# phylo42/RAPPAS

Measured on AMD Instinct MI355X. Metric: reads placed/sec (whole node), 150 bp DNA vs 10^7-kmer DB, higher is better.
Workload: dtype f32; 1 GPU; C2: DNA k=10, 999 branches, phylo-kmer DB of 786432 keys / 9995042 entries (seed 42), replicated per GPU; 10000000 x 150 symbol reads per GPU per step (uniform, seed 1+rank), keep_at_most=7; reads_per_gpu=10000000

## Files before the change

### rappas_amd/csrc/rk_engine.hip

```cpp
#include "rk_kernels.hip"
#include "rk_internal.h"
#include "rk_pack_host.h"
#include "rk_translate_host.h"
#include "rk_plan.h"
#include "rk_geometry.h"

#include <cmath>
#include <cstdarg>
#include <cstdio>
#include <cstdlib>
#include <algorithm>
#include <array>
#include <chrono>
#include <condition_variable>
#include <cstring>
#include <cerrno>
#include <cstddef>
#include <deque>
#include <functional>
#include <map>
#include <set>
#include <memory>
#include <atomic>
#include <mutex>
// ... 785 lines not shown
    }
    CL_TRY(hipDeviceSynchronize());
#undef CL_TRY
    db->compact_nib = src->compact_nib;
    finish_db(db, meta, src->info.table_mode, src->indexed, src->view.mono != 0, src->info.n_keys, src->info.n_entries, src->info.table_slots,
              src->view.hash_mask, table_bytes, blob_bytes, src->info.max_row_len);
    db->lanes_per_read = src->lanes_per_read;
    *out = db;
    return RK_OK;
    RK_GUARD_END("rk_db_clone")
}

extern "C" int rk_db_get_info(const rk_db *db, rk_db_info *info) {
    if (!db || !info) return fail(RK_ERR_INVALID, "rk_db_get_info: null argument");
    *info = db->info;
    return RK_OK;
}

extern "C" void *rk_host_alloc(uint64_t bytes) {
    void *p = nullptr;
    hipError_t e = hipHostMalloc(&p, bytes ? bytes : 1, hipHostMallocDefault);
    if (e != hipSuccess) {
        (void)fail(e == hipErrorOutOfMemory ? RK_ERR_NOMEM : RK_ERR_HIP, "rk_host_alloc(%llu) failed: %s", (unsigned long long)bytes, hipGetErrorString(e));
        return nullptr;
    }
    return p;
}

extern "C" void rk_host_free(void *p) {
    if (p) (void)hipHostFree(p);
}

extern "C" uint32_t rk_packed_words(const rk_db *db, uint32_t max_len) {
    if (!db) return 0;
    uint64_t bits = (uint64_t)max_len * db->info.bits_per_symbol;
    uint32_t w = (uint32_t)((bits + 31) / 32);
    return w ? w : 1;
}

extern "C" int rk_set_lanes_per_read(rk_db *db, uint32_t lanes) {
    if (!db) return fail(RK_ERR_INVALID, "rk_set_lanes_per_read: null db");
    if (lanes != 0 && lanes != 8 && lanes != 16 && lanes != 32 && lanes != 64)
        return fail(RK_ERR_INVALID, "rk_set_lanes_per_read: lanes must be 0 (auto), 8, 16, 32 or 64");
    if (lanes != 0 && db->indexed)
        return fail(RK_ERR_UNSUPPORTED, "rk_set_lanes_per_read: this database uses the large-tree image (n_branches > %u, long rows): always the workgroup-per-read kernel", RK_WG_MIN_BRANCHES);
    db->lanes_per_read = lanes;
    return RK_OK;
}

static int geometry_error(rk_geom::Status st, const rk_db *db, uint32_t keep_at_most = 0, size_t lds_per_read = 0) {
    switch (st) {
    case rk_geom::GEOM_OK: return RK_OK;
    case rk_geom::KEEP_NEEDS_LANES: return fail(RK_ERR_INVALID, "keep_at_most=%u needs lanes_per_read >= %u", keep_at_most, keep_at_most);
    case rk_geom::READ_EXCEEDS_LDS: return fail(RK_ERR_UNSUPPORTED, "n_branches=%u needs %zu B of LDS per read, more than one CU has (%zu B)", db->info.n_branches, lds_per_read, db->lds_per_cu);
    case rk_geom::NO_WG_WINDOW: return fail(RK_ERR_UNSUPPORTED, "n_branches=%u: no score-vector window fits one CU's LDS (%zu B)", db->info.n_branches, db->lds_per_cu);
    case rk_geom::WINDOWED_NO_FIT: return fail(RK_ERR_UNSUPPORTED, "internal: windowed geometry does not fit the LDS");
    default: return fail(RK_ERR_INVALID, "internal: ambiguity kernel launched without a score-vector geometry");
    }
}
static int db_geometry(const rk_db *db, uint32_t keep_at_most, Geometry &g) {
    const rk_geom::Status st = rk_geom::choose_geometry(db->info.n_branches, db->info.bits_per_symbol, db->lds_per_cu, db->lanes_per_read, keep_at_most, geom_knobs(), g);
    return geometry_error(st, db, keep_at_most, st == rk_geom::READ_EXCEEDS_LDS ? g.lds_per_wave : 0);
}
static int db_wg_geometry(const rk_db *db, WgGeometry &g, uint32_t keep_at_most = 16) {
    return geometry_error(rk_geom::choose_wg_geometry(db->info.n_branches, db->lds_per_cu, keep_at_most, geom_knobs(), g), db);
}

static bool use_pipelined16(const rk_db *db, const Geometry &g, const PlaceArgs &args) {
    static const bool off = rk_knob("RK_NO_PIPE") != nullptr;
    return !off && g.G == 16 && db->info.table_mode != RK_TABLE_HASH && db->info.rows_bytes < ROWS_FIT32_LIMIT && args.words_per_read <= 16;
}

template <int G, int BITS, int TM, bool WIDE>
static int launch_variant(const rk_db *db, const Geometry &g, const PlaceArgs &args, hipStream_t stream) {
    constexpr int PU = rk_geom::probe_unroll(G, BITS);
    constexpr int U = G == 64 ? RK_RING64 : RK_RING;
    auto kern = place_packed_kernel<G, BITS, TM, WIDE, U, PU>;
    decltype(kern) clade_kern = nullptr;
    PlaceArgs la = args;
    bool whole_simds = false;
    if constexpr (G == 16 && !WIDE && TM != TM_HASH) {
        if (use_pipelined16(db, g, args)) {
            whole_simds = TM == TM_COMPACT;
            auto k16 = place_packed16_kernel<BITS, TM, U, PU>;
            auto k24 = place_packed16_kernel<BITS, TM, U, PU, TM == TM_COMPACT>;
            if constexpr (BITS == 5) {
                if (!args.lens && args.fixed_len >= db->info.k && args.fixed_len - db->info.k + 1 <= 96u) {
                    k16 = place_packed16_kernel<BITS, TM, U, 6>;
                    k24 = place_packed16_kernel<BITS, TM, U, 6, TM == TM_COMPACT>;
                }
            }
            kern = k16;
            if (TM == TM_COMPACT && db->d_dense_rows) {
                kern = k24;
                la.db.compact = (const uint4 *)db->d_dense_table;
                la.db.rows = (const unsigned char *)db->d_dense_rows;
                la.db.rows_bytes = db->dense_rows_bytes;
                if (args.perm) {
                    clade_kern = k16;
                    la.only_if = 3u;
                }
            }
        }
    }
    const Grid grid{64, g.lds_per_wave, g.waves_per_cu, (args.n_reads + g.NG - 1) / g.NG, whole_simds};
    if (int rc = launch_grid(db->cu_count, kern, grid, stream, la)) return rc;
    if (!clade_kern) return RK_OK;
    PlaceArgs ca = args;
    ca.only_if = 4u;
    return launch_grid(db->cu_count, clade_kern, grid, stream, ca);
}

template <int G, int BITS>
static int launch_t(const rk_db *db, const Geometry &g, const PlaceArgs &a, hipStream_t s) {
    const bool wide = db->info.rows_bytes >= ROWS_FIT32_LIMIT;
    switch (db->info.table_mode) {
    case RK_TABLE_DIRECT: return wide ? launch_variant<G, BITS, TM_COMPACT, true>(db, g, a, s) : launch_variant<G, BITS, TM_COMPACT, false>(db, g, a, s);
    case RK_TABLE_DIRECT8: return wide ? launch_variant<G, BITS, TM_DIRECT8, true>(db, g, a, s) : launch_variant<G, BITS, TM_DIRECT8, false>(db, g, a, s);
    default: return wide ? launch_variant<G, BITS, TM_HASH, true>(db, g, a, s) : launch_variant<G, BITS, TM_HASH, false>(db, g, a, s);
    }
}
static bool use_windowed(const rk_db *db, uint32_t keep_at_most, uint32_t words_per_read) {
    static const bool off = rk_knob("RK_NO_WINDOW") != nullptr;
    const uint64_t max_symbols = (uint64_t)words_per_read * 32 / db->info.bits_per_symbol;
    const bool fits = words_per_read <= 16 || max_symbols * 9 <= db->info.n_branches || db->info.n_branches > 16000;
    return !off && db->windowed && db->lanes_per_read == 0 && keep_at_most <= 16 && fits;
}

static void *launch_scratch(const rk_db *db, hipStream_t s, size_t bytes) {
    std::lock_guard<std::mutex> lock(db->scratch_mu);
    rk_db::LaunchScratch *b = nullptr;
    for (auto &x : db->scratch)
        if (x.s == s) { b = &x; break; }
    if (!b) {
        if (db->scratch.size() >= 16) {
            auto lru = std::min_element(db->scratch.begin(), db->scratch.end(), [](const rk_db::LaunchScratch &x, const rk_db::LaunchScratch &y) { return x.used < y.used; });
            hipStreamCaptureStatus cs = hipStreamCaptureStatusNone;
            if (hipStreamIsCapturing(s, &cs) != hipSuccess || cs != hipStreamCaptureStatusNone || hipDeviceSynchronize() != hipSuccess) {
                (void)hipGetLastError();
                return nullptr;
            }
            if (lru->p) (void)hipFree(lru->p);
            db->scratch.erase(lru);
        }
        db->scratch.push_back({s, nullptr, 0, 0});
        b = &db->scratch.back();
    }
    b->used = ++db->scratch_clock;
    if (b->cap < bytes) {
        hipStreamCaptureStatus cs = hipStreamCaptureStatusNone;
        if (hipStreamIsCapturing(s, &cs) != hipSuccess || cs != hipStreamCaptureStatusNone) {
            (void)hipGetLastError();
            return nullptr;
        }
        if (b->p) {
            if (hipStreamSynchronize(s) != hipSuccess) { (void)hipGetLastError(); return nullptr; }
            (void)hipFree(b->p);
            b->p = nullptr;
            b->cap = 0;
        }
        const size_t want = ((bytes + bytes / 4) + ((size_t)1 << 20) - 1) & ~(((size_t)1 << 20) - 1);
        if (hipMalloc(&b->p, want) != hipSuccess || !b->p) {
            (void)hipGetLastError();
            b->p = nullptr;
            return nullptr;
        }
        b->cap = want;
    }
    return b->p;
}

struct TileOrder {
// ... 661 lines not shown
```

### rappas_amd/csrc/rk_geometry.h

```cpp
#pragma once
#include <cstddef>
#include <cstdint>
#include <initializer_list>
#include "rk_plan.h"

#ifndef RK_WG_MIN_BRANCHES
#define RK_WG_MIN_BRANCHES 8192u
#endif
#ifndef RK_WG_MIN_MEAN_ROW
#define RK_WG_MIN_MEAN_ROW 320.0
#endif
#ifndef RK_WG_ALWAYS_BRANCHES
#define RK_WG_ALWAYS_BRANCHES 65535u
#endif
#ifndef RK_WINDOW_MIN_BRANCHES
#define RK_WINDOW_MIN_BRANCHES 1276u
#endif
#ifndef RK_RING
#define RK_RING 8
#endif
#ifndef RK_RING64
#define RK_RING64 8
#endif

namespace rk_geom {

enum Status { GEOM_OK = 0, KEEP_NEEDS_LANES, READ_EXCEEDS_LDS, NO_WG_WINDOW, WINDOWED_NO_FIT, NO_SCORE_VECTOR };
struct Knobs {
    uint32_t list_cap = 0, waves_per_cu = 0;
    int wg_passes = 1;
    uint32_t hash_waves = ~0u;
    bool window_always = false, wstream_always = false;
};
constexpr uint32_t ROW_ENTRIES = 16;

static inline uint64_t resident_per_cu(uint64_t by_lds, uint64_t by_query, size_t lds) {
    uint64_t out = by_lds < by_query ? by_lds : by_query;
    if (lds) {
        const uint64_t by_granule = (160ull * 1024) / ((lds + 511) & ~(size_t)511);
        if (by_granule >= 1 && by_granule < out) out = by_granule;
    }
    return out;
}
static inline uint64_t grid_blocks(int cu_count, uint64_t per_cu, uint64_t work) { return (uint64_t)cu_count * per_cu > work ? work : (uint64_t)cu_count * per_cu; }

struct Geometry { uint32_t G, NG, s_stride, list_cap, pu; size_t lds_per_wave; uint32_t waves_per_cu; };
static constexpr uint32_t probe_unroll(uint32_t G, uint32_t bits) { return G <= 16 ? (bits == 5 && G == 16 ? 7 : 9) : (G == 32 ? 5 : 3); }
static inline Status choose_geometry(uint32_t nb, uint32_t bits, size_t lds_per_cu, uint32_t lanes_per_read, uint32_t keep_at_most, const Knobs &kn, Geometry &g) {
    const uint32_t s_stride = (nb + 4) & ~3u;
    const size_t target = lds_per_cu / 8;
    const size_t fixed = (size_t)s_stride * 4;
    auto bytes_for = [&](uint32_t G, uint32_t cap) { return (size_t)(64 / G) * (fixed + (size_t)cap * 8); };
    uint32_t G = lanes_per_read;
    if (G == 0) {
        G = 64;
        if (keep_at_most <= 16 && bytes_for(16, 16 + 3 * RK_RING + 40) <= lds_per_cu / 6) G = 16;
        else if (keep_at_most <= 32 && bytes_for(32, 32 + 3 * RK_RING + 40) <= lds_per_cu / 4) G = 32;
    }
    if (G < keep_at_most) return KEEP_NEEDS_LANES;
    const uint32_t NG = 64 / G, pu = probe_unroll(G, bits);
    const uint32_t min_cap = G + 3 * (G == 64 ? RK_RING64 : RK_RING) + 40;
    size_t per_group_target = target / NG;
    uint32_t cap = min_cap;
    if (per_group_target > fixed + (size_t)min_cap * 8) {
        size_t c = (per_group_target - fixed) / 8;
        cap = (uint32_t)(c > 256 ? 256 : c);
        if (cap < min_cap) cap = min_cap;
    }
    if (kn.list_cap >= min_cap && kn.list_cap <= 4096) cap = kn.list_cap;
    cap &= ~1u;
    g.G = G; g.NG = NG; g.s_stride = s_stride; g.list_cap = cap; g.pu = pu;
    g.lds_per_wave = bytes_for(G, cap);
    if (g.lds_per_wave > lds_per_cu) return READ_EXCEEDS_LDS;
    uint32_t w = (uint32_t)(lds_per_cu / g.lds_per_wave);
    g.waves_per_cu = w > 32 ? 32 : w;
    if (kn.waves_per_cu >= 1 && kn.waves_per_cu < g.waves_per_cu) g.waves_per_cu = kn.waves_per_cu;
    return GEOM_OK;
}

constexpr uint32_t RK_MAX_WINDOWS = 64;
static inline unsigned char winspec_byte(uint32_t first, uint32_t last) {
    const uint32_t span = last - first;
    return (unsigned char)(first | ((span < 3u ? span : 3u) << 6));
}
constexpr uint64_t RK_WINDOW_MAX_BLOB = 1ull << 31;
static inline bool windows_pay(uint32_t nb, uint64_t blob_units, uint64_t space, const Knobs &kn) {
    if (kn.window_always) return true;
    return 5 * blob_units <= 11 * space || nb > RK_WG_MIN_BRANCHES;
}
struct WindowPlan {
    uint32_t W = 0, n_win = 0, s_stride = 0, main_cap = 0, work_cap = 0;
    bool stream = false;
    double units_per_code = 0.0;
};
#ifndef RK_WSTREAM_MIN_BRANCHES
#define RK_WSTREAM_MIN_BRANCHES 4500u
#endif
static inline bool wstream_tree(uint32_t nb, uint32_t bits, double units_per_code, double units_per_row, const Knobs &kn) {
    if (kn.wstream_always) return true;
    if (150.0 * units_per_code > RK_WSTREAM_MAX_UNITS) return false;
    if (units_per_row > 2.5) return false;
    return bits == 5 || nb > RK_WSTREAM_MIN_BRANCHES;
}
static inline bool window_plan(uint32_t nb, uint32_t bits, double units_per_code, double units_per_row, const Knobs &kn, WindowPlan &wp) {
    if (nb <= RK_WINDOW_MIN_BRANCHES || nb > RK_WG_ALWAYS_BRANCHES) return false;
    wp.stream = wstream_tree(nb, bits, units_per_code, units_per_row, kn);
    wp.units_per_code = units_per_code;
    uint32_t n_win = wp.stream ? (nb + 511) / 512 : (nb + 895) / 896;
    if (n_win > RK_MAX_WINDOWS) n_win = RK_MAX_WINDOWS;
    wp.n_win = n_win;
    wp.W = ((nb + n_win - 1) / n_win + 3) & ~3u;
    wp.s_stride = wp.W + 4;
    const uint32_t per_group_words = 160 * 1024 / 8 / 4 / 4;
    const uint32_t avail = per_group_words - wp.s_stride;
    uint32_t work = avail > 256 + 88 ? avail - 256 : 88;
    if (work > 200) work = 200;
    wp.work_cap = work & ~1u;
    wp.main_cap = (avail - wp.work_cap) & ~1u;
    if (wp.main_cap > 640) wp.main_cap = 640;
    return wp.main_cap >= 160;
}
struct ImageKind { bool indexed, windowable; };
static inline ImageKind image_kind(uint32_t nb, uint32_t bits, bool direct, uint64_t space, uint64_t slot_units, uint32_t max_len, double mean_len, const Knobs &kn) {
    WindowPlan wp;
    const bool dense64_ahead = nb > RK_WG_MIN_BRANCHES && ((nb <= 9900u && mean_len >= 200.0 && mean_len < 1200.0) || (nb <= 13300u && mean_len >= 250.0 && mean_len < 750.0));
    const bool windowable = (!dense64_ahead || kn.window_always) && window_plan(nb, bits, space ? (double)slot_units / (double)space : 0.0, mean_len / ROW_ENTRIES + 0.5, kn, wp) && direct &&
                            (max_len + ROW_ENTRIES - 1) / ROW_ENTRIES <= 255 && slot_units * 128 < RK_WINDOW_MAX_BLOB && windows_pay(nb, slot_units, space, kn);
    const bool long_rows = mean_len >= RK_WG_MIN_MEAN_ROW;
    const bool indexed = nb > RK_WG_MIN_BRANCHES && ((long_rows && !dense64_ahead) || (!windowable && !dense64_ahead && nb > 16000u));
    return {indexed, windowable && !indexed};
}
struct WaveGeometry {
    uint32_t s_stride = 0, main_cap = 0, work_cap = 0, list_cap = 0, waves_cu = 0;
    size_t lds_wave = 0;
    bool wide = false;
};
static inline size_t lds_of_four_reads(uint32_t s_stride, uint32_t main_cap, uint32_t work_cap) { return (size_t)4 * (s_stride + main_cap + work_cap) * 4; }
static inline Status waves_that_fit(size_t lds_per_cu, uint32_t max_waves, WaveGeometry &o) {
    o.lds_wave = lds_of_four_reads(o.s_stride, o.main_cap, o.work_cap);
    o.waves_cu = (uint32_t)(lds_per_cu / o.lds_wave);
    if (o.waves_cu < 1) return WINDOWED_NO_FIT;
    if (o.waves_cu > max_waves) o.waves_cu = max_waves;
    return GEOM_OK;
}

static inline Status windowed_geometry(const WindowPlan &plan, uint32_t keep_at_most, uint32_t words_per_read, size_t lds_per_cu, WaveGeometry &o) {
    const uint32_t work_min = keep_at_most > 8 ? 96u : 88u;
    o.work_cap = plan.work_cap < work_min || words_per_read > 10 ? work_min : plan.work_cap;
    o.main_cap = plan.main_cap + plan.work_cap - o.work_cap;
    o.s_stride = plan.s_stride; o.list_cap = o.work_cap / 2;
    return waves_that_fit(lds_per_cu, 8u, o);
}

static inline bool sorted_wide(const WindowPlan &wp) { return wp.W > 512; }
static inline Status sorted_geometry(const WindowPlan &wp, size_t lds_per_cu, WaveGeometry &o) {
    const uint32_t work_min = 96u;
    const uint32_t ring = 8u;
    uint32_t work = work_min > 64u + 3u * ring ? work_min : 64u + 3u * ring;
    work = (work + 1) & ~1u;
    const uint32_t need = 200 + 5 * wp.n_win + 3 * ring;
    const uint32_t s_str = wp.W + 16;
// ... 89 lines not shown
```

### rappas_amd/csrc/rk_kernels.hip

```cpp
#include "rk_device.h"
#include "rk_slots24.h"
#include "rk_compact32.h"
#include "rk_translate.h"
#include "rk_masses.h"
#include "rk_samples.h"
#include "rk_epca.h"
#include "rk_edpl.h"
#include "rk_kmeans.h"
#include "rk_diversity.h"

#include <type_traits>
#ifndef RK_ROW_NT
#define RK_ROW_NT 0
#endif
#ifndef RK_ROW_AUX
#define RK_ROW_AUX 0
#endif
#ifndef RK_HEADS_MAX_K
#define RK_HEADS_MAX_K 16
#endif
#ifndef RK_ABLATE
#define RK_ABLATE 0
#endif
#include "../../include/rappas_place.h"

namespace rk {

#ifdef RK_STAMPS
__device__ unsigned long long rk_stamp_buf[2 * 4096 * 16];
__device__ __forceinline__ unsigned long long rk_now() {
    unsigned long long t;
    __builtin_amdgcn_sched_barrier(0);
    asm volatile("s_memtime %0\n\ts_waitcnt lgkmcnt(0)" : "=s"(t)::"memory");
    __builtin_amdgcn_sched_barrier(0);
    return t;
}
struct Stamps {
    unsigned long long st_[16] = {0, 0, 0, 0, 0, 0, 0, 0, 0, 0, 0, 0, 0, 0, 0, 0};
    unsigned long long t_ = rk_now();
    __device__ __forceinline__ void mark(int slot) {
        const unsigned long long n_ = rk_now();
        st_[slot] += n_ - t_;
        t_ = n_;
    }
    __device__ __forceinline__ void add(int slot, unsigned long long n) { st_[slot] += n; }
    __device__ __forceinline__ Stamps *ptr() { return this; }
    __device__ __forceinline__ void store(unsigned long long index) const {
        for (int i = 0; i < 16; i++) rk_stamp_buf[index * 16 + i] = st_[i];
    }
};
#else
struct Stamps {
    __device__ __forceinline__ void mark(int) {}
    __device__ __forceinline__ void add(int, unsigned long long) {}
    __device__ __forceinline__ Stamps *ptr() { return nullptr; }
    __device__ __forceinline__ void store(unsigned long long) const {}
};
#endif

__device__ __forceinline__ u32 ord_f32(float f) {
    u32 u = __float_as_uint(f);
    return (u & 0x80000000u) ? ~u : (u | 0x80000000u);
}
__device__ __forceinline__ float unord_f32(u32 o) {
    u32 u = (o & 0x80000000u) ? (o & 0x7FFFFFFFu) : ~o;
    return __uint_as_float(u);
}
__device__ __forceinline__ u64 make_key(u32 raw_score_bits, u32 branch) {
    return ((u64)ord_f32(__uint_as_float(raw_score_bits)) << 32) | (u64)(0xFFFFu - branch);
}
__device__ __forceinline__ u64 shfl64(u64 v, int src, int width) {
    u32 lo = (u32)v, hi = (u32)(v >> 32);
    lo = __shfl(lo, src, width);
    hi = __shfl(hi, src, width);
    return ((u64)hi << 32) | lo;
}
__device__ __forceinline__ u64 shfl_xor64(u64 v, int m, int width) {
    u32 lo = (u32)v, hi = (u32)(v >> 32);
    lo = __shfl_xor(lo, m, width);
    hi = __shfl_xor(hi, m, width);
    return ((u64)hi << 32) | lo;
}
__device__ __forceinline__ double shfl_f64(double v, int src, int width) {
    return __longlong_as_double((long long)shfl64((u64)__double_as_longlong(v), src, width));
}
__device__ __forceinline__ bool tile_order_given(const PlaceArgs &a) { return a.perm != nullptr && *a.keep_order == 0u; }
__device__ __forceinline__ u32 batch_class(const PlaceArgs &a) { return a.keep_order[0] == 0u ? 2u : (a.keep_order[3] != 0u ? 1u : 0u); }
__device__ __forceinline__ bool batch_is_mine(const PlaceArgs &a) {
    if (!a.only_if || !a.perm) return true;
    return ((a.only_if >> batch_class(a)) & 1u) != 0u;
}
__device__ __forceinline__ bool takes_only_marked(const PlaceArgs &a) {
// ... 362 lines not shown
    }
}

constexpr u32 ITEM_FILLER = 0xFFFFFF00u;
typedef u32 v2u32 __attribute__((ext_vector_type(2)));

__device__ __forceinline__ __amdgpu_buffer_rsrc_t rows_resource(const DbView &db) {
    return __builtin_amdgcn_make_buffer_rsrc((void *)db.rows, (short)0, (int)(u32)db.rows_bytes, 0x00020000);
}

template <int G, int U, bool MONO, bool WIN = false, bool D24 = false>
__device__ __forceinline__ void accumulate_units(u32 *S, const u32 *items, int wcnt, u32 li,
                                                 __amdgpu_buffer_rsrc_t rs, float QT, float T, u32 wlo4p4 = 4u, u32 w4 = 0xFFFFFFFFu) {
    static_assert(!D24 || (G == 16 && !WIN), "dense units: 16-lane groups, whole trees");
    static_assert(rk_slots24::SLOT_BITS == SLOT24_BITS, "rk_slots24.h unpacks the slot words rk_device.h defines");
    const u32 li8 = li * 8;
    const u32 my_unit = li >> 4;
    const rk_slots24::Shifts sh24 = rk_slots24::lane_shifts(li);
    u32 sb[U], it[U];
    float sc[U];
    auto issue = [&](u32 item, u32 &b, float &v) {
        u32 off = item + li8;
        if (G > 16) off = (my_unit <= (item & 7u)) ? (item & ~127u) + li8 : ITEM_FILLER;
        if (RK_ABLATE & 16) off = li8;
        const v2u32 e = __builtin_amdgcn_raw_buffer_load_b64(rs, (int)off, 0, RK_ROW_AUX);
        b = e.x;
        v = __uint_as_float(e.y);
    };
    auto slot_of = [&](u32 b) {
        if (!WIN) return b;
        const u32 t = b - wlo4p4;
        return (t < w4) ? t + 4u : 0u;
    };
    auto prepare = [&](float v, u32 *&pa, u32 *&pb) {
        const int w = (int)__float_as_uint(v);
        const u32 r = (u32)__builtin_amdgcn_update_dpp(w, w, 0x128, 0xF, 0x3, false);
        const rk_slots24::Slots s = rk_slots24::lane_slots(sh24, r);
        pa = S + s.a;
        pb = S + s.b;
    };
#pragma unroll
    for (int u = 0; u < U; u++) issue(items[u], sb[u], sc[u]);
#pragma unroll
    for (int u = 0; u < U; u++) it[u] = items[U + u];
    int s0 = 0;
    if (D24) {
        u32 *pa, *pb;
        prepare(sc[0], pa, pb);
        while (true) {
#pragma unroll
            for (int u = 0; u < U; u++) {
                u32 *na, *nb;
                if (RK_ABLATE & 8) {
                    asm volatile("" ::"v"(pa), "v"(pb), "v"(sb[u]), "v"(sc[u]));
                    prepare(sc[(u + 1) % U], na, nb);
                } else {
                    const u32 oa = *pa, ob = *pb;
                    prepare(sc[(u + 1) % U], na, nb);
                    *pa = __float_as_uint(touch_base<MONO>(oa, QT) + __uint_as_float(sb[u]));
                    *pb = __float_as_uint(touch_base<MONO>(ob, QT) + sc[u]);
                }
                issue(it[u], sb[u], sc[u]);
                it[u] = items[s0 + 2 * U + u];
                pa = na;
                pb = nb;
            }
            s0 += U;
            if (s0 >= wcnt) break;
        }
        return;
    }
    while (true) {
#pragma unroll
        for (int u = 0; u < U; u++) {
            apply_slot<MONO>(S, slot_of(sb[u]), sc[u], QT, T);
            issue(it[u], sb[u], sc[u]);
            it[u] = items[s0 + 2 * U + u];
        }
        s0 += U;
        if (s0 >= wcnt) break;
    }
}

template <int U>
struct UnitRing {
    u32 sb[U], it[U];
    float sc[U];
};
template <int G>
__device__ __forceinline__ u32 unit_offset(u32 item, u32 li) {
    const u32 li8 = li * 8;
    u32 off = item + li8;
    if (G > 16) off = ((li >> 4) <= (item & 7u)) ? (item & ~127u) + li8 : ITEM_FILLER;
    if (RK_ABLATE & 16) off = li8;
    return off;
}
__device__ __forceinline__ void unit_load(__amdgpu_buffer_rsrc_t rs, u32 off, u32 &b, float &v) {
    const v2u32 e = __builtin_amdgcn_raw_buffer_load_b64(rs, (int)off, 0, RK_ROW_AUX);
    b = e.x;
    v = __uint_as_float(e.y);
}
template <int G>
__device__ __forceinline__ void unit_issue(__amdgpu_buffer_rsrc_t rs, u32 item, u32 li, u32 &b, float &v) {
    unit_load(rs, unit_offset<G>(item, li), b, v);
}
typedef __attribute__((address_space(3))) const u32 *lds_cu32;
template <bool MONO, bool FEED>
__device__ __forceinline__ float touch_base_behind(u32 old, float QT, const u32 *na, const u32 *nb, u32 off) {
    const lds_cu32 la = (lds_cu32)na, lb = (lds_cu32)nb;
    float base;
    if (MONO) {
        if (FEED) asm("v_max_f32 %0, %1, %2" : "=v"(base) : "v"(old), "v"(QT), "v"(la), "v"(lb), "v"(off));
        else asm("v_max_f32 %0, %1, %2" : "=v"(base) : "v"(old), "v"(QT), "v"(la), "v"(lb));
    } else {
        if (FEED) asm("" : "+v"(old) : "v"(la), "v"(lb), "v"(off));
        else asm("" : "+v"(old) : "v"(la), "v"(lb));
        base = touch_base<false>(old, QT);
    }
    return base;
}
template <int G, int U>
__device__ __forceinline__ void units_issue(UnitRing<U> &r, const u32 *items, u32 li, __amdgpu_buffer_rsrc_t rs) {
#pragma unroll
    for (int u = 0; u < U; u++) unit_issue<G>(rs, items[u], li, r.sb[u], r.sc[u]);
#pragma unroll
    for (int u = 0; u < U; u++) r.it[u] = items[U + u];
}
template <int F, int N, bool B> struct StepBlock { static constexpr int first = F, steps = N; static constexpr bool feed = B; };
template <int G, int U, bool MONO, bool WIN = false, bool D24 = false, bool TILE = false>
__device__ __forceinline__ void units_run(UnitRing<U> &r, u32 *S, const u32 *items, int wcnt, u32 li, __amdgpu_buffer_rsrc_t rs, float QT, float T,
                                          u32 wlo4p4 = 4u, u32 w4 = 0xFFFFFFFFu, Stamps *stamps = nullptr) {
    static_assert(!D24 || (G == 16 && !WIN), "dense units: 16-lane groups, whole trees");
    static_assert(!TILE || U == 8, "a tail of up to three pairs of steps");
    static_assert(rk_slots24::SLOT_BITS == SLOT24_BITS, "rk_slots24.h unpacks the slot words rk_device.h defines");
    const rk_slots24::Shifts sh24 = rk_slots24::lane_shifts(li);
    const u32 li8 = li * 8;
    u32(&sb)[U] = r.sb;
    u32(&it)[U] = r.it;
    float(&sc)[U] = r.sc;
    auto issue = [&](u32 item, u32 &b, float &v) { unit_issue<G>(rs, item, li, b, v); };
    auto slot_of = [&](u32 b) {
        if (!WIN) return b;
        const u32 t = b - wlo4p4;
        return (t < w4) ? t + 4u : 0u;
    };
    auto prepare = [&](float v, u32 *&pa, u32 *&pb) {
        u32 r;
        asm volatile("v_mov_b32 %0, %1\n\ts_nop 1\n\tv_mov_b32_dpp %0, %1 row_ror:8 row_mask:0xf bank_mask:0x3" : "=&v"(r) : "v"(v));
        const rk_slots24::Slots s = rk_slots24::lane_slots(sh24, r);
        pa = S + s.a;
        pb = S + s.b;
    };
    if (stamps) {
        asm volatile("" ::"v"(sc[0]));
        stamps->mark(7);
    }
    int s0 = 0;
    u32 *pa = S, *pb = S;
    if (D24) prepare(sc[0], pa, pb);
    auto block = [&](auto kind) __attribute__((always_inline)) {
        constexpr int F = decltype(kind)::first, N = decltype(kind)::steps;
        constexpr bool FEED = decltype(kind)::feed;
#pragma unroll
        for (int u = F; u < F + N; u++) {
            if (D24) {
                u32 *na = pa, *nb = pb;
                if (RK_ABLATE & 8) {
                    asm volatile("" ::"v"(pa), "v"(pb), "v"(sb[u]), "v"(sc[u]));
                    prepare(sc[(u + 1) % U], na, nb);
                } else {
                    const u32 oa = *pa, ob = *pb;
                    prepare(sc[(u + 1) % U], na, nb);
                    u32 off = 0u;
                    if (FEED && (RK_ABLATE & 16)) off = unit_offset<G>(it[u], li);
                    else if (FEED) asm volatile("v_add_u32 %0, %1, %2" : "=v"(off) : "v"(it[u]), "v"(li8));
                    *pa = __float_as_uint(touch_base_behind<MONO, FEED>(oa, QT, na, nb, off) + __uint_as_float(sb[u]));
                    *pb = __float_as_uint(touch_base_behind<MONO, FEED>(ob, QT, na, nb, off) + sc[u]);
                    if (FEED) unit_load(rs, off, sb[u], sc[u]);
                }
                pa = na;
                pb = nb;
                if (FEED) {
                    if (RK_ABLATE & 8) issue(it[u], sb[u], sc[u]);
                    it[u] = items[s0 + 2 * U + u];
                }
                continue;
            }
            apply_slot<MONO>(S, slot_of(sb[u]), sc[u], QT, T);
            if (FEED) {
                issue(it[u], sb[u], sc[u]);
                it[u] = items[s0 + 2 * U + u];
            }
        }
    };
    if (TILE) {
        while (wcnt - s0 > U - 2) {
            block(StepBlock<0, U, true>());
            s0 += U;
        }
        const int left = wcnt - s0;
        if (left > 0) {
            block(StepBlock<0, 2, false>());
            if (left > 2) {
                block(StepBlock<2, 2, false>());
                if (left > 4) block(StepBlock<4, 2, false>());
            }
        }
        if (stamps) stamps->add(12, (unsigned long long)(s0 + (left > 0 ? (left + 1) & ~1 : 0)));
        return;
    }
    while (true) {
        block(StepBlock<0, U, true>());
        s0 += U;
        if (s0 >= wcnt) break;
    }
    if (stamps) stamps->add(12, (unsigned long long)s0);
}
template <int S>
__device__ __forceinline__ u32 row_ror32(u32 v) {
    return (u32)__builtin_amdgcn_update_dpp(0, (int)v, 0x120 + S, 0xF, 0xF, false);
}
template <int G, int S>
__device__ __forceinline__ u64 group_rotate(u64 v, u32 li) {
    if (G == 16) {
        return ((u64)row_ror32<S>((u32)(v >> 32)) << 32) | row_ror32<S>((u32)v);
    } else {
        return shfl64(v, (int)((li + G - S) % G), G);
    }
}
template <int G, int S>
struct RankAbove {
    static __device__ __forceinline__ int run(u64 v, u32 li) {
        return ((group_rotate<G, S>(v, li) > v) ? 1 : 0) + RankAbove<G, S - 1>::run(v, li);
    }
};
template <int G>
struct RankAbove<G, 0> {
    static __device__ __forceinline__ int run(u64, u32) { return 0; }
};
template <int G>
__device__ __forceinline__ u64 group_max(u64 v) {
    if (G == 16) {
        u64 o;
        o = ((u64)row_ror32<8>((u32)(v >> 32)) << 32) | row_ror32<8>((u32)v); v = o > v ? o : v;
        o = ((u64)row_ror32<4>((u32)(v >> 32)) << 32) | row_ror32<4>((u32)v); v = o > v ? o : v;
        o = ((u64)row_ror32<2>((u32)(v >> 32)) << 32) | row_ror32<2>((u32)v); v = o > v ? o : v;
        o = ((u64)row_ror32<1>((u32)(v >> 32)) << 32) | row_ror32<1>((u32)v); v = o > v ? o : v;
        return v;
    } else {
#pragma unroll
        for (int s = 1; s < G; s <<= 1) {
            u64 o = shfl_xor64(v, s, G);
            v = o > v ? o : v;
        }
        return v;
    }
}

template <int G>
__device__ __forceinline__ int rank_candidates(const u64 *list, int c, u64 *win, int K, u32 li) {
    if (c <= G) {
        const u64 mine = ((int)li < c) ? list[li] : 0ull;
        const int rank = RankAbove<G, G - 1>::run(mine, li);
        if (mine != 0 && rank < K) win[rank] = mine;
    } else {
        for (int j = (int)li; j < c; j += G) {
            const u64 mine = list[j];
            int rank = 0;
            for (int t = 0; t < c; t++) rank += (list[t] > mine) ? 1 : 0;
            if (rank < K) win[rank] = mine;
        }
    }
    wave_lds_fence();
    return c < K ? c : K;
}

template <int G>
__device__ __forceinline__ int select_topk_scan(u32 *S, u32 ns, u32 li, u32 gi, int K, u64 *list, int cap, u64 &win_key, Stamps &stamps) {
    const u32 nb = ns;
    u64 *win = list + (cap - 16);
    const int capc = cap - 16;
    const uint4 *S4 = (const uint4 *)S;
    uint4 *S4w = (uint4 *)S;
    const u32 n4 = (nb + 3) / 4;
    float mo = -INFINITY;
    u32 mi = 0xFFFFFFFFu;
    for (u32 q = li; q < n4; q += G) {
        const uint4 v4 = S4[q];
// ... 726 lines not shown
struct Batch0Words<PU, PU> {
    static __device__ __forceinline__ void run(u32 recw, u32 (&w)[PU + 1]) { w[PU] = row_bcast32<(PU < 16 ? PU : 15)>(recw); }
};

template <int BITS, int PU>
__device__ __forceinline__ void record_codes(u32 recw, u32 pos, u32 li, u32 k, u32 Q, u64 (&code)[PU]) {
    if (BITS == 2 && PU <= 15) {
        if (pos == 0) {
            u32 w[PU + 1];
            Batch0Words<PU, 0>::run(recw, w);
            const u32 mask = (k >= 16) ? 0xFFFFFFFFu : ((1u << (2 * k)) - 1u);
#pragma unroll
            for (int u = 0; u < PU; u++) code[u] = __builtin_amdgcn_alignbit(w[u + 1], w[u], 2 * li) & mask;
            return;
        }
    }
#pragma unroll
    for (int u = 0; u < PU; u++) {
        const u32 j0 = pos + u * 16 + li;
        const u32 j = j0 < Q ? j0 : 0u;
        const u32 bit = j * BITS, wi = bit >> 5, sh = bit & 31;
        const u32 w0 = __shfl(recw, (int)(wi & 15u), 16);
        u32 w1 = __shfl(recw, (int)((wi + 1) & 15u), 16);
        w1 = wi + 1 < 16 ? w1 : 0u;
        const u32 nbits = k * BITS;
        if (nbits <= 32) {
            const u32 c32 = __builtin_amdgcn_alignbit(w1, w0, sh);
            code[u] = nbits == 32 ? c32 : (c32 & ((1u << nbits) - 1u));
            continue;
        }
        u32 w2 = 0u;
        if (BITS * 12 + 31 > 64) {
            w2 = __shfl(recw, (int)((wi + 2) & 15u), 16);
            w2 = (wi + 2 < 16 && nbits + sh > 64) ? w2 : 0u;
        }
        const u64 c = funnel96(w0, w1, w2, sh);
        code[u] = nbits >= 64 ? c : (c & ((1ull << nbits) - 1));
    }
}

template <int BITS, int PU>
__device__ __forceinline__ void record_indices(u32 recw, u32 pos, u32 li, u32 k, u32 Q, u32 (&idx)[PU]) {
    if (BITS == 2) {
        const u32 mask = (k >= 16) ? 0xFFFFFFFFu : ((1u << (2 * k)) - 1u);
        if (PU <= 15 && pos == 0) {
            u32 w[PU + 1];
            Batch0Words<PU, 0>::run(recw, w);
#pragma unroll
            for (int u = 0; u < PU; u++) idx[u] = __builtin_amdgcn_alignbit(w[u + 1], w[u], 2 * li) & mask;
            return;
        }
#pragma unroll
        for (int u = 0; u < PU; u++) {
            const u32 j0 = pos + u * 16 + li;
            const u32 j = j0 < Q ? j0 : 0u;
            const u32 wi = j >> 4, sh = (j & 15u) * 2u;
            const u32 w0 = __shfl(recw, (int)(wi & 15u), 16);
            u32 w1 = __shfl(recw, (int)((wi + 1) & 15u), 16);
            w1 = wi + 1 < 16 ? w1 : 0u;
            idx[u] = __builtin_amdgcn_alignbit(w1, w0, sh) & mask;
        }
        return;
    }
    u64 code[PU];
    record_codes<BITS, PU>(recw, pos, li, k, Q, code);
#pragma unroll
    for (int u = 0; u < PU; u++) idx[u] = (u32)dense_index<BITS>(code[u], k);
}

template <int PU, bool C32>
struct ProbeBatch {
    RawSlot raw[PU];
    u32 j[C32 ? PU : 1];
    u64 code[C32 ? 1 : PU];
};
template <int PU, bool C32>
struct RowBatch {
    u32 unit[C32 ? PU : 1], n[C32 ? PU : 1];
    u64 desc[C32 ? 1 : PU];
};
__device__ __forceinline__ u64 unit_desc(u32 unit, u32 n) { return n ? ((u64)(unit * ROW_UNIT) << DESC_LEN_BITS) | (u64)(n * ROW_UNIT) : 0ull; }

template <int BITS, int TM, int U, int PU, bool D24 = false>
__global__ void __launch_bounds__(256) place_packed16_kernel(PlaceArgs a) {
    constexpr int G = 16, NG = 4;
    static_assert(TM != TM_HASH, "direct tables only");
    static_assert(!D24 || TM == TM_COMPACT, "the dense view carries a compact table");
    if (!batch_is_mine(a)) return;
    extern __shared__ u32 lds[];
    const bool perm_given = tile_order_given(a);
    const u32 lane = threadIdx.x & 63;
    const u32 wave = threadIdx.x >> 6;
    const u32 waves_per_block = blockDim.x >> 6;
    const u32 gi = lane / G, li = lane % G;
    const u32 wave_words = NG * (a.s_stride + 2 * a.list_cap);
    u32 *wbase = lds + wave * wave_words;
    u32 *S = wbase + gi * a.s_stride;
    u64 *list = (u64 *)(wbase + NG * a.s_stride) + gi * a.list_cap;
    u32 *items = (u32 *)list;
    const u32 nb = a.db.n_branches;
    const u32 k = a.db.k;
    const float T = a.db.T;
    const __amdgpu_buffer_rsrc_t rows_rs = rows_resource(a.db);
    const int cap_items = (int)(a.list_cap * 2) - 3 * U - 2;
    const int cap_rows = (int)a.list_cap - 1;
    const u32 wpr = a.words_per_read;

    for (u32 i = li; i < a.s_stride; i += G) S[i] = S_UNTOUCHED;
    wave_lds_fence();

    const u64 n_tiles = (a.n_reads + NG - 1) / NG;
    const u64 wave_global = (u64)blockIdx.x * waves_per_block + wave;
    const u64 wave_count = (u64)gridDim.x * waves_per_block;

    auto load_tile = [&](u64 tile, u32 &recw, u32 &R, u32 &fin, bool &have) {
        const u64 slot = tile * NG + gi;
        have = tile < n_tiles && slot < a.n_reads;
        const u64 r = have ? tile_read(a, slot, perm_given) : 0ull;
        recw = 0; R = 0; fin = 0;
        if (have) {
            if (li < wpr) recw = a.packed[r * wpr + li];
            R = a.lens ? a.lens[r] : a.fixed_len;
            fin = a.flags_in ? a.flags_in[r] : 0u;
        }
    };
    constexpr bool C32 = TM == TM_COMPACT;
    const bool nib = a.db.compact_nib != 0;
    auto fetch_batch = [&](u32 recw, u32 pos, u32 Q, ProbeBatch<PU, C32> &pb) {
        if constexpr (C32) {
            u32 idx[PU];
            record_indices<BITS, PU>(recw, pos, li, k, Q, idx);
            const unsigned char *table = (const unsigned char *)a.db.compact;
#pragma unroll
            for (int u = 0; u < PU; u++) {
                const rk_compact32::Pos p = nib ? rk_compact32::locate_nib(idx[u]) : rk_compact32::locate_byte(idx[u]);
                pb.j[u] = p.j;
                pb.raw[u].v = *(const uint4 *)(table + p.blk * 16u);
            }
        } else {
            record_codes<BITS, PU>(recw, pos, li, k, Q, pb.code);
#pragma unroll
            for (int u = 0; u < PU; u++) pb.raw[u] = lookup_fetch<BITS, TM>(a.db, pb.code[u]);
        }
    };
    auto decode_batch = [&](const ProbeBatch<PU, C32> &pb, u32 pos, u32 Q, RowBatch<PU, C32> &rows) {
        if constexpr (C32) {
#pragma unroll
            for (int u = 0; u < PU; u++) {
                const uint4 v = pb.raw[u].v;
                const rk_compact32::Row r = nib ? rk_compact32::decode_nib(v.x, v.y, v.z, v.w, pb.j[u]) : rk_compact32::decode_byte(v.x, v.y, v.z, v.w, pb.j[u]);
                rows.unit[u] = r.unit;
                rows.n[u] = r.n;
            }
        } else {
#pragma unroll
            for (int u = 0; u < PU; u++) {
                const u32 j = pos + u * G + li;
                const u64 d = lookup_decode<BITS, TM>(a.db, pb.raw[u], pb.code[u]);
                rows.desc[u] = j < Q ? d : 0ull;
            }
        }
    };

    Stamps stamps;
    u32 c_recw, c_R, c_fin;
    bool c_have;
    RowBatch<PU, C32> rows0;
    {
        load_tile(wave_global, c_recw, c_R, c_fin, c_have);
        ProbeBatch<PU, C32> pb;
        const u32 Q0 = read_head<BITS>(a, c_R, c_fin, c_have).Q;
        fetch_batch(c_recw, 0u, Q0, pb);
        decode_batch(pb, 0u, Q0, rows0);
    }

    for (u64 tile = wave_global; tile < n_tiles; tile += wave_count) {
        const bool have = c_have;
        const u64 r = have ? tile_read(a, tile * NG + gi, perm_given) : 0ull;
        const u32 fin = c_fin;
        const ReadHead h = read_head<BITS>(a, c_R, fin, have);
        const u32 Q = h.Q;
        const float QT = h.QT;

        int cnt = 0;
        UnitRing<U> ring;
        bool ring_live = false;
        constexpr bool EARLY = D24;
        auto flush = [&]() __attribute__((always_inline)) {
            int wcnt = __builtin_amdgcn_readlane(cnt, 0);
            wcnt = max(wcnt, __builtin_amdgcn_readlane(cnt, 32));
            wcnt = max(wcnt, __builtin_amdgcn_readlane(cnt, 16));
            wcnt = max(wcnt, __builtin_amdgcn_readlane(cnt, 48));
            for (int i = cnt + (int)li; i < wcnt + 2 * U; i += G) items[i] = ITEM_FILLER;
            wave_lds_fence();
            stamps.mark(10);
            if (!ring_live) units_issue<G, U>(ring, items, li, rows_rs);
            ring_live = false;
            stamps.mark(11);
            if (a.db.mono) units_run<G, U, true, false, D24, true>(ring, S, items, wcnt, li, rows_rs, QT, T, 4u, 0xFFFFFFFFu, stamps.ptr());
            else units_run<G, U, false, false, D24, true>(ring, S, items, wcnt, li, rows_rs, QT, T, 4u, 0xFFFFFFFFu, stamps.ptr());
            stamps.mark(4);
            wave_lds_fence();
            stamps.mark(10);
            cnt = 0;
        };
        auto emit_batch = [&](const RowBatch<PU, C32> &rows, u32 pos, bool more) {
            u32 nch[PU], excl[PU], rb[PU];
            int total = 0;
            bool wide_rows = false;
            bool early = false;
#pragma unroll
            for (int u = 0; u < PU; u++) {
                if constexpr (C32) nch[u] = pos + u * G + li < Q ? rows.n[u] : 0u;
                else nch[u] = (((u32)rows.desc[u] & DESC_LEN_MASK) + G - 1) >> 4;
                if constexpr (C32) rb[u] = rows.unit[u] * 128u;
                else rb[u] = (u32)(rows.desc[u] >> DESC_LEN_BITS) * 8u;
                if (!(C32 && nib)) wide_rows = wide_rows || nch[u] > 15u;
            }
            auto row_scan = [](u32 v) {
                v += (u32)__builtin_amdgcn_update_dpp(0, (int)v, 0x111, 0xF, 0xF, true);
                v += (u32)__builtin_amdgcn_update_dpp(0, (int)v, 0x112, 0xF, 0xF, true);
                v += (u32)__builtin_amdgcn_update_dpp(0, (int)v, 0x114, 0xF, 0xF, true);
                v += (u32)__builtin_amdgcn_update_dpp(0, (int)v, 0x118, 0xF, 0xF, true);
                return v;
            };
            auto write_rows = [&](int u_lo, int u_hi) {
#pragma unroll
                for (int u = u_lo; u < u_hi; u++) {
                    const int base = cnt + (int)excl[u];
                    if (nch[u] > 0) items[base] = rb[u];
                    if (nch[u] > 1) items[base + 1] = rb[u] + 128u;
                    for (u32 c = 2; __any(c < nch[u]); c++)
                        if (c < nch[u]) items[base + (int)c] = rb[u] + c * 128u;
                }
            };
            if (!__any(wide_rows)) {
#pragma unroll
                for (int u0 = 0; u0 < PU; u0 += 4) {
                    u32 packed = nch[u0];
                    if (u0 + 1 < PU) packed |= nch[u0 + 1 < PU ? u0 + 1 : u0] << 8;
                    if (u0 + 2 < PU) packed |= nch[u0 + 2 < PU ? u0 + 2 : u0] << 16;
                    if (u0 + 3 < PU) packed |= nch[u0 + 3 < PU ? u0 + 3 : u0] << 24;
                    const u32 incl = row_scan(packed);
                    const u32 tot = row_bcast32<15>(incl);
#pragma unroll
                    for (int b = 0; b < 4; b++) {
                        if (u0 + b < PU) {
                            const int u = u0 + b < PU ? u0 + b : u0;
                            excl[u] = (u32)total + ((incl >> (8 * b)) & 0xFFu) - nch[u];
                            total += (int)((tot >> (8 * b)) & 0xFFu);
                        }
                    }
                    if constexpr (EARLY) {
                        if (u0 == 0 && PU > 4 && pos == 0 && !__any(total < 2 * U || total > cap_items)) {
                            write_rows(0, 4);
                            wave_lds_fence();
                            units_issue<G, U>(ring, items, li, rows_rs);
                            __builtin_amdgcn_sched_barrier(0);
                            ring_live = early = true;
                        }
                    }
                }
            } else {
#pragma unroll
                for (int u = 0; u < PU; u++) {
                    const u32 incl = row_scan(nch[u]);
                    excl[u] = (u32)total + incl - nch[u];
                    total += (int)row_bcast32<15>(incl);
                }
            }
            if (!early && __any(more && cnt + total > cap_items)) flush();
            if (D24 && __any(more && total > cap_items)) {
                for (u32 done = 0; __any(done < (u32)total);) {
                    const u32 room = (u32)(cap_items - cnt);
#pragma unroll
                    for (int u = 0; u < PU; u++) {
                        for (u32 c = 0; __any(c < nch[u]); c++) {
                            const u32 x = excl[u] + c - done;
                            if (c < nch[u] && x < room) items[cnt + (int)x] = rb[u] + c * 128u;
                        }
                    }
                    const u32 take = min((u32)total - done, room);
                    cnt += (int)take;
                    done += take;
                    if (__any(done < (u32)total)) flush();
                }
            } else if (__any(more && total > cap_items)) {
                const int per_part = cap_rows / G;
                for (int u_lo = 0; u_lo < PU; u_lo += per_part) {
                    int rc = 0;
#pragma unroll
                    for (int u = 0; u < PU; u++) {
                        const bool part = u >= u_lo && u < u_lo + per_part;
                        const bool hit = part && nch[u] != 0;
                        const u64 bal = __ballot(hit);
                        const u64 sub = group_bits<G>(bal, gi);
                        u64 d;
                        if constexpr (C32) d = unit_desc(rows.unit[u], nch[u]);
                        else d = rows.desc[u];
                        if (hit) list[rc + count_below<G>(sub, li)] = d;
                        rc += __builtin_popcountll(sub);
                    }
                    if (li == 0) list[rc] = 0;
                    wave_lds_fence();
                    if (__any(rc > 0)) accumulate_list<G, U, false>(S, nb, list, rc, li, a.db.rows, QT, T);
                    wave_lds_fence();
                }
            } else {
                if (!early) write_rows(0, PU < 4 ? PU : 4);
                write_rows(PU < 4 ? PU : 4, PU);
                cnt += total;
            }
        };

        stamps.mark(0);
        emit_batch(rows0, 0u, Q > 0);
        for (u32 pos = PU * G; __any(pos < Q); pos += PU * G) {
            ProbeBatch<PU, C32> pb;
            RowBatch<PU, C32> rows;
            fetch_batch(c_recw, pos, Q, pb);
            __builtin_amdgcn_sched_barrier(0);
            decode_batch(pb, pos, Q, rows);
            emit_batch(rows, pos, pos < Q);
        }
        stamps.mark(2);
        load_tile(tile + wave_count, c_recw, c_R, c_fin, c_have);
        if (__any(cnt > 0)) flush();
        stamps.mark(4);
        ProbeBatch<PU, C32> npb;
        const u32 nQ = read_head<BITS>(a, c_R, c_fin, c_have).Q;
        fetch_batch(c_recw, 0u, nQ, npb);
        __builtin_amdgcn_sched_barrier(0);
        stamps.mark(1);

        u64 win_key;
        int numBest = 0;
        if (RK_ABLATE & 2) { win_key = list[0]; for (u32 i = li; i <= nb; i += G) S[i] = S_UNTOUCHED; }
        else numBest = select_topk<G>(S, nb, li, gi, (int)a.keep_at_most, list, (int)a.list_cap, win_key, stamps);
        wave_lds_fence();
        stamps.mark(5);
// ... 2196 lines not shown
```

Baseline: 433.9 million reads/s.

## Deepen dense-kernel load ring and hold ring items in row-broadcast lanes

New measurement: 442.3 million reads/s (median of 6 runs). 1.02x the previous value.

```diff
diff --git a/rappas_amd/csrc/rk_engine.hip b/rappas_amd/csrc/rk_engine.hip
--- a/rappas_amd/csrc/rk_engine.hip
+++ b/rappas_amd/csrc/rk_engine.hip
@@ -891,12 +891,14 @@
     if constexpr (G == 16 && !WIDE && TM != TM_HASH) {
         if (use_pipelined16(db, g, args)) {
             whole_simds = TM == TM_COMPACT;
+            constexpr bool D24 = TM == TM_COMPACT;
+            constexpr int U24 = D24 ? RK_RING_DENSE : U;
             auto k16 = place_packed16_kernel<BITS, TM, U, PU>;
-            auto k24 = place_packed16_kernel<BITS, TM, U, PU, TM == TM_COMPACT>;
+            auto k24 = place_packed16_kernel<BITS, TM, U24, PU, D24>;
             if constexpr (BITS == 5) {
                 if (!args.lens && args.fixed_len >= db->info.k && args.fixed_len - db->info.k + 1 <= 96u) {
                     k16 = place_packed16_kernel<BITS, TM, U, 6>;
-                    k24 = place_packed16_kernel<BITS, TM, U, 6, TM == TM_COMPACT>;
+                    k24 = place_packed16_kernel<BITS, TM, U24, 6, D24>;
                 }
             }
             kern = k16;
diff --git a/rappas_amd/csrc/rk_geometry.h b/rappas_amd/csrc/rk_geometry.h
--- a/rappas_amd/csrc/rk_geometry.h
+++ b/rappas_amd/csrc/rk_geometry.h
@@ -21,6 +21,9 @@
 #endif
 #ifndef RK_RING64
 #define RK_RING64 8
+#endif
+#ifndef RK_RING_DENSE
+#define RK_RING_DENSE 12
 #endif
 
 namespace rk_geom {
@@ -77,6 +80,8 @@
     if (kn.waves_per_cu >= 1 && kn.waves_per_cu < g.waves_per_cu) g.waves_per_cu = kn.waves_per_cu;
     return GEOM_OK;
 }
+static constexpr uint32_t dense_list_fillers(uint32_t U) { return U + 16 > 2 * U ? U + 16 : 2 * U; }
+static constexpr uint32_t dense_cap_items(uint32_t list_cap, uint32_t U) { return 2 * list_cap - dense_list_fillers(U) - 2; }
 
 constexpr uint32_t RK_MAX_WINDOWS = 64;
 static inline unsigned char winspec_byte(uint32_t first, uint32_t last) {
diff --git a/rappas_amd/csrc/rk_kernels.hip b/rappas_amd/csrc/rk_kernels.hip
--- a/rappas_amd/csrc/rk_kernels.hip
+++ b/rappas_amd/csrc/rk_kernels.hip
@@ -8,6 +8,7 @@
 #include "rk_edpl.h"
 #include "rk_kmeans.h"
 #include "rk_diversity.h"
+#include "rk_geometry.h"
 
 #include <type_traits>
 #ifndef RK_ROW_NT
@@ -536,9 +537,9 @@
     }
 }
 
-template <int U>
+template <int U, bool ROWIT = false>
 struct UnitRing {
-    u32 sb[U], it[U];
+    u32 sb[U], it[ROWIT ? 2 : U];
     float sc[U];
 };
 template <int G>
@@ -573,24 +574,46 @@
     }
     return base;
 }
-template <int G, int U>
-__device__ __forceinline__ void units_issue(UnitRing<U> &r, const u32 *items, u32 li, __amdgpu_buffer_rsrc_t rs) {
-#pragma unroll
-    for (int u = 0; u < U; u++) unit_issue<G>(rs, items[u], li, r.sb[u], r.sc[u]);
-#pragma unroll
-    for (int u = 0; u < U; u++) r.it[u] = items[U + u];
+#define RK_ROW_ITEM_CASE(L) \
+    case L: asm volatile("v_add_u32_dpp %0, %1, %2 row_newbcast:" #L " row_mask:0xf bank_mask:0xf" : "=v"(off) : "v"(row), "v"(li8)); break;
+__device__ __forceinline__ u32 row_item_offset(int place, u32 row, u32 li8) {
+    u32 off = 0u;
+    switch (place) {
+        RK_ROW_ITEM_CASE(0) RK_ROW_ITEM_CASE(1) RK_ROW_ITEM_CASE(2) RK_ROW_ITEM_CASE(3) RK_ROW_ITEM_CASE(4) RK_ROW_ITEM_CASE(5)
+        RK_ROW_ITEM_CASE(6) RK_ROW_ITEM_CASE(7) RK_ROW_ITEM_CASE(8) RK_ROW_ITEM_CASE(9) RK_ROW_ITEM_CASE(10) RK_ROW_ITEM_CASE(11)
+        RK_ROW_ITEM_CASE(12) RK_ROW_ITEM_CASE(13) RK_ROW_ITEM_CASE(14) RK_ROW_ITEM_CASE(15)
+    }
+    return off;
+}
+#undef RK_ROW_ITEM_CASE
+__device__ __forceinline__ void row_items_next(u32 &row, u32 next) { asm volatile("v_mov_b32 %0, %1\n\ts_nop 1" : "=v"(row) : "v"(next)); }
+template <int G, int U, bool ROWIT>
+__device__ __forceinline__ void units_issue(UnitRing<U, ROWIT> &r, const u32 *items, u32 li, __amdgpu_buffer_rsrc_t rs) {
+    if constexpr (ROWIT) {
+        static_assert(G == 16 && U <= 16, "a read's 16 lanes hold a block's items");
+        const u32 head = items[li];
+#pragma unroll
+        for (int u = 0; u < U; u++) unit_load(rs, (RK_ABLATE & 16) ? li * 8 : row_item_offset(u, head, li * 8), r.sb[u], r.sc[u]);
+        r.it[0] = items[U + li];
+    } else {
+#pragma unroll
+        for (int u = 0; u < U; u++) unit_issue<G>(rs, items[u], li, r.sb[u], r.sc[u]);
+#pragma unroll
+        for (int u = 0; u < U; u++) r.it[u] = items[U + u];
+    }
 }
 template <int F, int N, bool B> struct StepBlock { static constexpr int first = F, steps = N; static constexpr bool feed = B; };
-template <int G, int U, bool MONO, bool WIN = false, bool D24 = false, bool TILE = false>
-__device__ __forceinline__ void units_run(UnitRing<U> &r, u32 *S, const u32 *items, int wcnt, u32 li, __amdgpu_buffer_rsrc_t rs, float QT, float T,
+template <int G, int U, bool MONO, bool WIN = false, bool D24 = false, bool TILE = false, bool ROWIT = false>
+__device__ __forceinline__ void units_run(UnitRing<U, ROWIT> &r, u32 *S, const u32 *items, int wcnt, u32 li, __amdgpu_buffer_rsrc_t rs, float QT, float T,
                                           u32 wlo4p4 = 4u, u32 w4 = 0xFFFFFFFFu, Stamps *stamps = nullptr) {
     static_assert(!D24 || (G == 16 && !WIN), "dense units: 16-lane groups, whole trees");
-    static_assert(!TILE || U == 8, "a tail of up to three pairs of steps");
+    static_assert(!TILE || (U >= 8 && U <= 16 && U % 2 == 0), "a tail of up to seven pairs of steps");
+    static_assert(!ROWIT || (D24 && TILE), "items in the lanes of a register: the dense instances of place_packed16_kernel");
     static_assert(rk_slots24::SLOT_BITS == SLOT24_BITS, "rk_slots24.h unpacks the slot words rk_device.h defines");
     const rk_slots24::Shifts sh24 = rk_slots24::lane_shifts(li);
     const u32 li8 = li * 8;
     u32(&sb)[U] = r.sb;
-    u32(&it)[U] = r.it;
+    u32(&it)[ROWIT ? 2 : U] = r.it;
     float(&sc)[U] = r.sc;
     auto issue = [&](u32 item, u32 &b, float &v) { unit_issue<G>(rs, item, li, b, v); };
     auto slot_of = [&](u32 b) {
@@ -611,6 +634,7 @@
     }
     int s0 = 0;
     u32 *pa = S, *pb = S;
+    if constexpr (ROWIT) asm volatile("" : "+v"(it[0]));
     if (D24) prepare(sc[0], pa, pb);
     auto block = [&](auto kind) __attribute__((always_inline)) {
         constexpr int F = decltype(kind)::first, N = decltype(kind)::steps;
@@ -626,24 +650,36 @@
                     const u32 oa = *pa, ob = *pb;
                     prepare(sc[(u + 1) % U], na, nb);
                     u32 off = 0u;
-                    if (FEED && (RK_ABLATE & 16)) off = unit_offset<G>(it[u], li);
-                    else if (FEED) asm volatile("v_add_u32 %0, %1, %2" : "=v"(off) : "v"(it[u]), "v"(li8));
+                    if constexpr (ROWIT) {
+                        if (FEED) off = (RK_ABLATE & 16) ? li8 : row_item_offset(u, it[0], li8);
+                    } else {
+                        if (FEED && (RK_ABLATE & 16)) off = unit_offset<G>(it[u], li);
+                        else if (FEED) asm volatile("v_add_u32 %0, %1, %2" : "=v"(off) : "v"(it[u]), "v"(li8));
+                    }
                     *pa = __float_as_uint(touch_base_behind<MONO, FEED>(oa, QT, na, nb, off) + __uint_as_float(sb[u]));
                     *pb = __float_as_uint(touch_base_behind<MONO, FEED>(ob, QT, na, nb, off) + sc[u]);
                     if (FEED) unit_load(rs, off, sb[u], sc[u]);
                 }
                 pa = na;
                 pb = nb;
-                if (FEED) {
+                if constexpr (ROWIT) {
+                    if (FEED) {
+                        if (RK_ABLATE & 8) unit_load(rs, (RK_ABLATE & 16) ? li8 : row_item_offset(u, it[0], li8), sb[u], sc[u]);
+                        if (u == F) it[1] = items[s0 + 2 * U + (int)li];
+                        if (u == F + N - 1) row_items_next(it[0], it[1]);
+                    }
+                } else if (FEED) {
                     if (RK_ABLATE & 8) issue(it[u], sb[u], sc[u]);
                     it[u] = items[s0 + 2 * U + u];
                 }
                 continue;
             }
-            apply_slot<MONO>(S, slot_of(sb[u]), sc[u], QT, T);
-            if (FEED) {
-                issue(it[u], sb[u], sc[u]);
-                it[u] = items[s0 + 2 * U + u];
+            if constexpr (!ROWIT) {
+                apply_slot<MONO>(S, slot_of(sb[u]), sc[u], QT, T);
+                if (FEED) {
+                    issue(it[u], sb[u], sc[u]);
+                    it[u] = items[s0 + 2 * U + u];
+                }
             }
         }
     };
@@ -657,7 +693,19 @@
             block(StepBlock<0, 2, false>());
             if (left > 2) {
                 block(StepBlock<2, 2, false>());
-                if (left > 4) block(StepBlock<4, 2, false>());
+                if (left > 4) {
+                    block(StepBlock<4, 2, false>());
+                    if constexpr (U > 8) if (left > 6) {
+                        block(StepBlock<6, 2, false>());
+                        if constexpr (U > 10) if (left > 8) {
+                            block(StepBlock<8, 2, false>());
+                            if constexpr (U > 12) if (left > 10) {
+                                block(StepBlock<10, 2, false>());
+                                if constexpr (U > 14) if (left > 12) block(StepBlock<12, 2, false>());
+                            }
+                        }
+                    }
+                }
             }
         }
         if (stamps) stamps->add(12, (unsigned long long)(s0 + (left > 0 ? (left + 1) & ~1 : 0)));
@@ -1550,7 +1598,7 @@
 __device__ __forceinline__ u64 unit_desc(u32 unit, u32 n) { return n ? ((u64)(unit * ROW_UNIT) << DESC_LEN_BITS) | (u64)(n * ROW_UNIT) : 0ull; }
 
 template <int BITS, int TM, int U, int PU, bool D24 = false>
-__global__ void __launch_bounds__(256) place_packed16_kernel(PlaceArgs a) {
+__global__ void __launch_bounds__(256) __attribute__((amdgpu_waves_per_eu(D24 ? 2 : 1))) place_packed16_kernel(PlaceArgs a) {
     constexpr int G = 16, NG = 4;
     static_assert(TM != TM_HASH, "direct tables only");
     static_assert(!D24 || TM == TM_COMPACT, "the dense view carries a compact table");
@@ -1570,7 +1618,8 @@
     const u32 k = a.db.k;
     const float T = a.db.T;
     const __amdgpu_buffer_rsrc_t rows_rs = rows_resource(a.db);
-    const int cap_items = (int)(a.list_cap * 2) - 3 * U - 2;
+    constexpr int FILLERS = D24 ? (int)rk_geom::dense_list_fillers(U) : 2 * U;
+    const int cap_items = D24 ? (int)rk_geom::dense_cap_items(a.list_cap, U) : (int)(a.list_cap * 2) - 3 * U - 2;
     const int cap_rows = (int)a.list_cap - 1;
     const u32 wpr = a.words_per_read;
 
@@ -1651,7 +1700,7 @@
         const float QT = h.QT;
 
         int cnt = 0;
-        UnitRing<U> ring;
+        UnitRing<U, D24> ring;
         bool ring_live = false;
         constexpr bool EARLY = D24;
         auto flush = [&]() __attribute__((always_inline)) {
@@ -1659,14 +1708,14 @@
             wcnt = max(wcnt, __builtin_amdgcn_readlane(cnt, 32));
             wcnt = max(wcnt, __builtin_amdgcn_readlane(cnt, 16));
             wcnt = max(wcnt, __builtin_amdgcn_readlane(cnt, 48));
-            for (int i = cnt + (int)li; i < wcnt + 2 * U; i += G) items[i] = ITEM_FILLER;
+            for (int i = cnt + (int)li; i < wcnt + FILLERS; i += G) items[i] = ITEM_FILLER;
             wave_lds_fence();
             stamps.mark(10);
-            if (!ring_live) units_issue<G, U>(ring, items, li, rows_rs);
+            if (!ring_live) units_issue<G, U, D24>(ring, items, li, rows_rs);
             ring_live = false;
             stamps.mark(11);
-            if (a.db.mono) units_run<G, U, true, false, D24, true>(ring, S, items, wcnt, li, rows_rs, QT, T, 4u, 0xFFFFFFFFu, stamps.ptr());
-            else units_run<G, U, false, false, D24, true>(ring, S, items, wcnt, li, rows_rs, QT, T, 4u, 0xFFFFFFFFu, stamps.ptr());
+            if (a.db.mono) units_run<G, U, true, false, D24, true, D24>(ring, S, items, wcnt, li, rows_rs, QT, T, 4u, 0xFFFFFFFFu, stamps.ptr());
+            else units_run<G, U, false, false, D24, true, D24>(ring, S, items, wcnt, li, rows_rs, QT, T, 4u, 0xFFFFFFFFu, stamps.ptr());
             stamps.mark(4);
             wave_lds_fence();
             stamps.mark(10);
@@ -1723,7 +1772,7 @@
                         if (u0 == 0 && PU > 4 && pos == 0 && !__any(total < 2 * U || total > cap_items)) {
                             write_rows(0, 4);
                             wave_lds_fence();
-                            units_issue<G, U>(ring, items, li, rows_rs);
+                            units_issue<G, U, D24>(ring, items, li, rows_rs);
                             __builtin_amdgcn_sched_barrier(0);
                             ring_live = early = true;
                         }
```
